# lincbrain/Fibers.jl

Measured on AMD Instinct MI355X. Metric: Mvoxels/s fit (GQI ODF + peaks, 140^3 x 270-dir); Mpoints/s streamline in extra, higher is better.
Workload: dtype f32 (operands as 2 fp16 pieces = 23 bits on MFMA, 3 piece products, f32 accumulate); 1 GPU; gqi_rec + find_peaks + qa normalisation (gqi.jl:109-201), ONE 140x140x140 x 270-frame volume (18 x b=5 + 84 dirs x {1000,2000,3000}), sphere_642, all-ones mask; voxels=2744000, voxels_per_gpu=2744000, frames=270, odf_vertices=321, parallelism=single GPU

## Files before the change

### fibers.jl_amd/csrc/odf.hip

```cpp
#include <algorithm>
#include <cmath>
#include <type_traits>
#include <utility>

#include "common.h"

namespace {

typedef float f32x16 __attribute__((ext_vector_type(16)));

constexpr int KT = 16;
constexpr int WG_VOX = 128;

#include "odf_gemm_f32.inc"
#include "odf_fused_epilogue.inc"
#include "odf_gemm3.inc"
#include "odf_mask.inc"
#include "odf_peaks.inc"
#include "odf_post.inc"

}

struct fib_odf_plan {
    int device = 0;
// ... 217 lines not shown
        for (int d = 0; d < p->maxdeg; d++) { const int32_t u = nbr32[(size_t)v * p->maxdeg + d]; if (u >= 0) mine.push_back(u); }
        for (int d = 0; d < FIB_S642_DEG; d++) if (fib_s642_nbr[v][d] < FIB_S642_NVERT) ref.push_back(fib_s642_nbr[v][d]);
        std::sort(mine.begin(), mine.end());
        if (mine != ref) p->is_s642 = false;
    }
    p->fused = p->fused_shape && p->is_s642 && p->At3f.p != nullptr;
    p->dsi2 = p->dsi2_shape && p->is_s642 && p->At3f.p != nullptr && p->At3b.p != nullptr;
    std::vector<int32_t> nbr64(nbr);
    for (auto &u : nbr64) if (u == p->rows_pad) u = p->nvert;
    if ((rc = p->nbr64.alloc(nbr64.size())) != FIB_OK) return rc;
    FIB_HIP(hipMemcpy(p->nbr64.p, nbr64.data(), nbr64.size() * sizeof(int32_t), hipMemcpyHostToDevice));
    std::vector<float> v3((size_t)p->nvert * 3, 0.0f);
    if (verts)
        for (int v = 0; v < p->nvert; v++)
            for (int c = 0; c < 3; c++) v3[3 * v + c] = verts[v + (size_t)nverts * c];
    if ((rc = p->At.alloc(At.size())) != FIB_OK) return rc;
    std::vector<uint32_t> effbits((size_t)p->Kpad / KT, 0u);
    for (int k = 0; k < K; k++) { if (frame_eff[k] != 0.0f) effbits[k / KT] |= 1u << (k % KT); else p->has_ineff = true; }
    if ((rc = p->effbits.alloc(effbits.size())) != FIB_OK) return rc;
    if ((rc = p->verts.alloc(v3.size())) != FIB_OK) return rc;
    if ((rc = p->nbr.alloc(nbr.size())) != FIB_OK) return rc;
    if ((rc = p->maxenc.alloc(4)) != FIB_OK) return rc;
    if ((rc = p->live_counts.alloc(4)) != FIB_OK) return rc;
    if ((rc = p->tickets.alloc(4)) != FIB_OK) return rc;
    FIB_HIP(hipMemset(p->tickets.p, 0, 4 * sizeof(unsigned)));
    if ((rc = p->selctr.alloc(2)) != FIB_OK) return rc;
    FIB_HIP(hipMemset(p->selctr.p, 0, 2 * sizeof(unsigned)));
    if ((rc = p->sellist.alloc(POST_SELCAP)) != FIB_OK) return rc;
    FIB_HIP(hipMemset(p->sellist.p, 0, POST_SELCAP * sizeof(unsigned long long)));
    if ((rc = p->odfmax.alloc(2)) != FIB_OK) return rc;
    FIB_HIP(hipMemcpy(p->At.p, At.data(), At.size() * sizeof(float), hipMemcpyHostToDevice));
    FIB_HIP(hipMemcpy(p->effbits.p, effbits.data(), effbits.size() * sizeof(uint32_t), hipMemcpyHostToDevice));
    FIB_HIP(hipMemcpy(p->verts.p, v3.data(), v3.size() * sizeof(float), hipMemcpyHostToDevice));
    FIB_HIP(hipMemcpy(p->nbr.p, nbr.data(), nbr.size() * sizeof(int32_t), hipMemcpyHostToDevice));
    return FIB_OK;
}

int check_plan_args(const float *bval, const float *bvec, int nvol, const float *verts, int nverts,
                    const int32_t *faces, int nfaces, fib_odf_plan **plan) {
    FIB_CHECK(plan != nullptr, FIB_ERR_INVALID, "plan output pointer is NULL");
    *plan = nullptr;
    FIB_CHECK(bval != nullptr && nvol > 0, FIB_ERR_MISSING_BVAL, "Missing b-value table from input DWI structure");
    FIB_CHECK(bvec != nullptr, FIB_ERR_MISSING_BVEC, "Missing gradient table from input DWI structure");
    FIB_CHECK(verts && faces && nverts >= 2 && nverts % 2 == 0 && nfaces > 0, FIB_ERR_INVALID, "invalid ODF tessellation");
    FIB_CHECK(nverts / 2 < 32768, FIB_ERR_UNSUPPORTED, "too many ODF vertices");
    return FIB_OK;
}

// ... 123 lines not shown

extern "C" int fib_odf_plan_matrix(const fib_odf_plan *plan, float *A, int *nrows, int *nvol, int *nvert) try {
    FIB_CHECK(plan != nullptr, FIB_ERR_INVALID, "plan is NULL");
    if (nrows) *nrows = plan->nrows;
    if (nvol) *nvol = plan->nvol;
    if (nvert) *nvert = plan->nvert;
    if (A) memcpy(A, plan->A.data(), plan->A.size() * sizeof(float));
    return FIB_OK;
} FIB_API_CATCH

namespace {

constexpr int FOLD_MB_MAX = 10;
template <int MB, int NX>
void launch_gemm(const GemmArgs &ga, unsigned grid, hipStream_t st) {
    if (ga.At3) {
        int ncu = 256, dev = 0;
        (void)hipGetDevice(&dev);
        (void)hipDeviceGetAttribute(&ncu, hipDeviceAttributeMultiprocessorCount, dev);
        GemmArgs g2 = ga;
        const int nw = 8;
        const int64_t items = fib::cdiv(ga.nvox, nw * 32) * ga.ntile_m;
        unsigned pg = (unsigned)std::min<int64_t>((int64_t)ncu * (8 / nw), items);
        pg = (pg + 7) / 8 * 8;
        auto go = [&](auto h2_) {
            constexpr bool H2 = decltype(h2_)::value;
            if (ga.fold) {
                if constexpr (MB <= FOLD_MB_MAX) hipLaunchKernelGGL((odf_gemm3_kernel<MB, NX, 8, true, false, H2>), dim3(pg), dim3(512), 0, st, g2);
                return;
            }
            if constexpr (MB == 10 && NX == 1) {
                if (ga.mean_hi) { hipLaunchKernelGGL((odf_gemm3_kernel<10, 1, 8, false, true, H2>), dim3(pg), dim3(512), 0, st, g2); return; }
            }
            hipLaunchKernelGGL((odf_gemm3_kernel<MB, NX, 8, false, false, H2>), dim3(pg), dim3(512), 0, st, g2);
        };
        if (ga.h2) go(std::true_type{}); else go(std::false_type{});
    }
    else hipLaunchKernelGGL((odf_gemm_kernel<MB, NX>), dim3(grid), dim3(256), 0, st, ga);
}

size_t peaks_smem(const fib_odf_plan *p) {
    return ((size_t)(p->rows_pad + 1) * PV + (size_t)PG * PV * PREC) * sizeof(float);
}

template <int DEG, bool EXACT>
int launch_peaks_t(const PeakArgs &pa, size_t smem, unsigned grid, hipStream_t st) {
// ... 135 lines not shown
    { const char *pi = fib::ab_env("FIBERS_PHASE_ITEM"); ga.phase_item = pi ? atoi(pi) : 2; }
    { const char *pw = fib::ab_env("FIBERS_PHASE_WG"); ga.phase_wg = pw ? atoi(pw) : 8; }
#endif
    ga.vec_ok = (nvox % 4 == 0 && ((uintptr_t)odf & 15) == 0 && (pdf == nullptr || ((uintptr_t)pdf & 15) == 0)) ? 1 : 0; ga.vidx = plan->live_vox.p; ga.nlive = plan->live_counts.p; ga.mask = mask; ga.effbits = plan->effbits.p;
    ga.out0 = pdf; ga.out1 = odf; ga.nvox = nvox;
    if (ga.At3 && plan->Gdev.p) {
        int rci = plan->inf_list.ensure((size_t)nvox);
        if (rci != FIB_OK) return rci;
        ga.fix_count = plan->live_counts.p + 2; ga.fix_list = plan->inf_list.p; ga.fix_cap = (int)std::min<int64_t>(nvox, INT32_MAX);
    }
    const bool sep = (flags & FIB_ODF_SEPARATE_PEAKS) != 0;
    const bool fuse = plan->fused && ga.At3 != nullptr && ga.vec_ok && !sep;
    {
        int rcm = plan->mean_hi.ensure((size_t)nvox + 4);
        if (rcm != FIB_OK) return rcm;
    }
    auto setup_fused = [&]() -> int {
        int rcf = plan->redo_list.ensure((size_t)nvox);
        if (rcf != FIB_OK) return rcf;
        ga.At3 = plan->At3f.p; ga.Aextra = plan->Aextraf.p;
        for (int k = 0; k < 3; k++) { ga.peak[k] = peak[k]; ga.qa[k] = qa[k]; }
        ga.verts = plan->verts.p; ga.maxenc = plan->maxenc.p; ga.mean_hi = plan->mean_hi.p;
        ga.redo_count = plan->live_counts.p + 3; ga.redo_list = plan->redo_list.p; ga.redo_cap = (int)std::min<int64_t>(nvox, INT32_MAX);
        { const char *pa = fib::ab_env("FIBERS_ODF_ANTI"); ga.anti = pa ? atoi(pa) : 3; }
        return FIB_OK;
    };
    if (fuse) { int rcf = setup_fused(); if (rcf != FIB_OK) return rcf; }
    ga.K = plan->gK; ga.Kpad = plan->Kpad; ga.M = plan->gM; ga.nrow0 = plan->gRow0; ga.ntile_m = plan->ntile_m;
    const bool fold_ok = plan->folded && ga.At3 != nullptr && plan->Kpad <= FKMAX && plan->scale_frame_raw >= 0 &&
                         (int64_t)plan->fold_span_max * nvox * 4 < (int64_t)0xE0000000ll;
    const bool fuse_fold = fold_ok && plan->MB <= FOLD_MB_MAX;
    const bool dsi2 = plan->dsi2 && fold_ok && ga.vec_ok && !sep;
    if (dsi2) {
        int rcf = setup_fused();
        if (rcf != FIB_OK) return rcf;
        ga.At3b = plan->At3b.p;
        ga.ntile_m = 2;
    }
    if (fuse_fold || dsi2) {
        ga.fold = 1;
        ga.rowA = plan->foldA.p; ga.rowB = plan->foldB.p;
    } else if (plan->folded) {
        int rcf = plan->folded_dwi.ensure((size_t)plan->gK * nvox);
        if (rcf != FIB_OK) return rcf;
        fib::ProfScope prof("dsi_fold", st);
        if (nvox % 4 == 0 && ((uintptr_t)dwi & 15) == 0 && ((uintptr_t)mask & 3) == 0)
// ... 136 lines not shown
    FIB_HIP(hipGetLastError());
    return FIB_OK;
} FIB_API_CATCH

extern "C" int fibd_qa_normalize_pair(float *const qa[3], int64_t nvox, float *odfmax_pair_dev, void *stream) try {
    FIB_CHECK(qa && qa[0] && qa[1] && qa[2] && odfmax_pair_dev && nvox > 0, FIB_ERR_INVALID, "NULL argument");
    hipLaunchKernelGGL(qa_normalize_kernel, dim3(2048), dim3(256), 0, (hipStream_t)stream, qa[0], qa[1], qa[2], nvox, odfmax_pair_dev, 0.0f, 1);
    FIB_HIP(hipGetLastError());
    return FIB_OK;
} FIB_API_CATCH

extern "C" int fibd_find_peaks(const fib_odf_plan *plan, const float *odf, int64_t nvox,
                               int32_t *isort_top, int32_t *nvalid, void *stream) try {
    FIB_CHECK(plan && odf && isort_top && nvalid && nvox > 0, FIB_ERR_INVALID, "NULL argument");
    fib::DeviceGuard guard;
    FIB_HIP(hipSetDevice(plan->device));
    return launch_peaks(plan, odf, nvox, nvox, nullptr, nullptr, isort_top, nvalid, false, (hipStream_t)stream);
} FIB_API_CATCH

#ifdef FIB_CLOCK_STAMP
extern "C" int fib_debug_clock_stamps(unsigned long long *out, int cap) try {
    FIB_CHECK(out && cap > 0 && cap <= 2048, FIB_ERR_INVALID, "invalid stamp buffer");
    FIB_HIP(hipDeviceSynchronize());
    FIB_HIP(hipMemcpyFromSymbol(out, HIP_SYMBOL(fib_clock_stamps), (size_t)cap * 4 * sizeof(unsigned long long), 0, hipMemcpyDeviceToHost));
    return FIB_OK;
} FIB_API_CATCH
extern "C" int fib_debug_phase_stamps(unsigned long long *out) try {
    FIB_CHECK(out, FIB_ERR_INVALID, "invalid stamp buffer");
    FIB_HIP(hipDeviceSynchronize());
    FIB_HIP(hipMemcpyFromSymbol(out, HIP_SYMBOL(fib_phase_stamps), sizeof(unsigned long long) * 512, 0, hipMemcpyDeviceToHost));
    return FIB_OK;
} FIB_API_CATCH

extern "C" int fib_debug_clock_clear(void) try {
    static unsigned long long zeros[2048][4];
    FIB_HIP(hipMemcpyToSymbol(HIP_SYMBOL(fib_clock_stamps), zeros, sizeof(zeros), 0, hipMemcpyHostToDevice));
    return FIB_OK;
} FIB_API_CATCH
#endif

extern "C" int fibd_find_peaks_work(const fib_odf_plan *plan, const float *odf, int64_t nvox,
                                    float *odf_peak, int32_t *isort, int32_t *nvalid, void *stream) try {
    FIB_CHECK(plan && odf && odf_peak && isort && nvalid && nvox > 0, FIB_ERR_INVALID, "NULL argument");
    FIB_CHECK(plan->nbr64.p != nullptr && plan->maxdeg > 0, FIB_ERR_INVALID, "the plan has no tessellation");
    fib::DeviceGuard guard;
    FIB_HIP(hipSetDevice(plan->device));
    const size_t smem = (size_t)plan->nvert * sizeof(unsigned long long) + (size_t)(plan->nvert + 1) * sizeof(float);
    FIB_CHECK(smem <= 64 * 1024, FIB_ERR_UNSUPPORTED, "ODF with %d vertices does not fit the peak finder's LDS", plan->nvert);
    const unsigned grid = (unsigned)std::min<int64_t>(nvox, 8192);
    hipLaunchKernelGGL(odf_peaks_work_kernel, dim3(grid), dim3(256), smem, (hipStream_t)stream, odf, nvox, nvox, plan->nvert, plan->deg_pad,
                       plan->nbr64.p, odf_peak, isort, nvalid);
    FIB_HIP(hipGetLastError());
    return FIB_OK;
} FIB_API_CATCH
```

### fibers.jl_amd/csrc/odf_fused_epilogue.inc

```

#include "sphere642_fused.inc"
#ifndef FIB_EPI_VARIANT
#define FIB_EPI_VARIANT 0
#endif
__device__ const short fib_f642_pos_vertex_dev[321] = {
#define FIB_F642_COPY(...) __VA_ARGS__
    FIB_F642_POS_LIST(FIB_F642_COPY)
};
__device__ const short fib_f642_slot_vertex_dev[2 * 161] = {
    FIB_F642_SLOT_LIST(FIB_F642_COPY)
#undef FIB_F642_COPY
};
constexpr int FQ_CAP = 10;
constexpr int FQ_LIST = FQ_CAP * 512;
constexpr int FQ_CAPB = 9;
constexpr int FQ_LISTB = FQ_CAPB * 320;
constexpr int FQ_NPOS = 320, FQ_NSLOT = 2 * 161, FQ_NV = 321;
constexpr int FQ_TABB = (2 * FQ_NPOS + FQ_NSLOT + 3 * FQ_NV) * 4 + 12;
static_assert(FQ_TABB % 16 == 0, "table block keeps the LDS carve-up 16-byte aligned");

__device__ __forceinline__ float fq_xhalf(float x, int kh) {
    const auto r = __builtin_amdgcn_permlane32_swap(__float_as_uint(x), __float_as_uint(x), false, false);
    return __uint_as_float(kh ? r[0] : r[1]);
}
__device__ __forceinline__ float fq_xhalf_max(float x) {
    const auto r = __builtin_amdgcn_permlane32_swap(__float_as_uint(x), __float_as_uint(x), false, false);
    return __builtin_fmaxf(__uint_as_float(r[0]), __uint_as_float(r[1]));
}
__device__ __forceinline__ float fq_max3(float a, float b, float c) { return __builtin_fmaxf(__builtin_fmaxf(a, b), c); }
__device__ __forceinline__ float fq_max3z(float a, float b) { return __builtin_fmaxf(__builtin_fmaxf(a, b), 0.0f); }
__device__ __forceinline__ float fq_min3(float a, float b, float c) { return __builtin_fminf(__builtin_fminf(a, b), c); }
__device__ __forceinline__ float fq_max2(float a, float b) { return __builtin_fmaxf(a, b); }

template <int NW, bool PRE = false, bool SCALE = false, bool POW2 = false, bool DRAIN = false, int TRN = 2, bool LB = false, int CAP = FQ_CAP>
__device__ __forceinline__ void gemm3_epilogue_fused(const GemmArgs &a, f32x16 (&acc)[10], float xrow, float vmax, float vnf, bool inb, bool lv,
                                                     int64_t vox, int lane, char *tr, char *lst, const uint64_t *posoff, const int *slotv, const float *vl,
                                                     unsigned &en_run, float scale = 1.0f, float xscale = 1.0f) {
    const int col = lane & 31, kh = lane >> 5;
    const float pm = fmaxf(vmax, __shfl_xor(vmax, 32));
    const float pn = vnf + __shfl_xor(vnf, 32);
    const bool nonfinite = pn != pn;
    const bool valid = lv && (pm > 0.0f || nonfinite);
    const bool refix = a.fix_list != nullptr && lv && pm == INFINITY;
    if (!PRE) xrow += __shfl_xor(xrow, 32);
    if constexpr (SCALE) {
#pragma unroll
        for (int m = 0; m < 10; m++)
#pragma unroll
            for (int r = 0; r < 16; r++) {
                if constexpr (POW2) asm("v_mul_legacy_f32 %0, %1, %2" : "=v"(acc[m][r]) : "v"(acc[m][r]), "v"(valid ? scale : 0.0f));
                else acc[m][r] = valid ? acc[m][r] * scale : 0.0f;
            }
        xrow = valid ? xrow * xscale : 0.0f;
    } else if (!__all(valid && !nonfinite)) {
#pragma unroll
        for (int m = 0; m < 10; m++)
#pragma unroll
            for (int r = 0; r < 16; r++) acc[m][r] = valid ? acc[m][r] : 0.0f;
        xrow = valid ? xrow : 0.0f;
    }
// ... 68 lines not shown
                const unsigned cw = m < 2 ? cw0 : m < 4 ? cw1 : m < 6 ? cw2 : m < 8 ? cw3 : cw4;
                unsigned byte = (cw >> (8 * (3 - (2 * (m & 1) + hb)))) & 0xffu;
#if FIB_EPI_VARIANT & 2
                {
                    const int b = 31 - __clz((int)(byte | 1u));
                    const int j = 7 - b;
                    const float x = tw[(8 * (j >> 2) + 2 * (j & 3)) * 32];
                    if (byte != 0u) { if (cnt < CAP) list_put(cnt, x, (uint32_t)(16 * m + 8 * hb + j)); cnt++; }
                    byte &= ~(1u << b);
                }
#endif
                if (__any(byte != 0u)) {
                    while (byte != 0u) {
                        const int b = 31 - __clz((int)byte);
                        byte &= ~(1u << b);
                        const int j = 7 - b;
                        const float x = tw[(8 * (j >> 2) + 2 * (j & 3)) * 32];
                        if (cnt < CAP) list_put(cnt, x, (uint32_t)(16 * m + 8 * hb + j));
                        cnt++;
                    }
                }
            }
        };
        if constexpr (DRAIN) __builtin_amdgcn_s_waitcnt(0x0F70);
        if (__all(qinb)) rows_out(std::false_type{}); else rows_out(std::true_type{});
        if (inb && kh == 0) a.out1[(int64_t)FIB_F642_POLE * a.stride + vox] = xrow;
        if (cpole) { if (cnt < CAP) list_put(cnt, xrow, 160u); cnt++; }
    }
    float vmin = INFINITY;
#if FIB_EPI_VARIANT & 1
    float vs0 = 0.0f, vs1 = 0.0f;
#pragma unroll
    for (int m = 0; m < 10; m++)
#pragma unroll
        for (int r = 0; r < 16; r += 2) {
            vmin = fq_min3(vmin, acc[m][r], acc[m][r + 1]);
            asm("v_add_f32 %0, %1, %0" : "+v"(vs0) : "v"(acc[m][r]));
            asm("v_add_f32 %0, %1, %0" : "+v"(vs1) : "v"(acc[m][r + 1]));
        }
    const float vsum = vs0 + vs1;
#else
    f32x2 vs2 = {0.0f, 0.0f};
#pragma unroll
    for (int m = 0; m < 10; m++)
#pragma unroll
        for (int r = 0; r < 16; r += 2) {
            vmin = fq_min3(vmin, acc[m][r], acc[m][r + 1]);
// ... 52 lines not shown
```

### fibers.jl_amd/csrc/odf_gemm3.inc

```

typedef __bf16 bf16x8_t __attribute__((ext_vector_type(8)));
typedef _Float16 f16x8_t __attribute__((ext_vector_type(8)));
typedef _Float16 f16x2_t __attribute__((ext_vector_type(2)));
typedef uint32_t u32x4_t __attribute__((ext_vector_type(4)));

__device__ __forceinline__ uint32_t cvt_pk_bf16(float lo, float hi) {
    uint32_t r;
    asm("v_cvt_pk_bf16_f32 %0, %1, %2" : "=v"(r) : "v"(lo), "v"(hi));
    return r;
}

constexpr int FKMAX = 512, FSMAX = FKMAX / KT;
template <int MB, int NX, int NW, bool FOLD, bool FUSE, bool H2, bool ONE = false>
constexpr int gemm3_lds_bytes() {
    constexpr bool SF = H2 && FOLD && ONE;
    return 2 * (H2 ? 2 : 3) * MB * 1024 + NW * (FUSE && !SF ? 4096 : 2048) + (NX > 0 ? (FUSE ? 2048 : 8192) : 0) +
           (FOLD ? 2 * FKMAX * 4 + 4 * FSMAX * 4 + (FUSE ? 0 : 2 * FKMAX * 4) : 0) + (FUSE ? NW * (SF ? FQ_LISTB : FQ_LIST) + FQ_TABB : 0) +
           (H2 && FUSE && !FOLD ? NW * (4096 + 512) : 0) +
           (SF ? NW * (8192 + 256) : 0);
}
template <int MB, int NX, int NW, bool FOLD = false, bool FUSE = false, bool ONE = false, bool H2 = false>
__device__ __forceinline__ void gemm3_body(const GemmArgs &a, char *lds) {
    static_assert(!FUSE || (MB == 10 && NX == 1), "the fused peak scan is generated for 10 blocks + 1 extra row");
    constexpr int NPIECE = (H2 ? 2 : 3) * MB;
    constexpr int TILEB = NPIECE * 1024;
    constexpr int NA = (NPIECE + NW - 1) / NW;
    constexpr int WGV = NW * 32;
    constexpr int NXA = NX > 0 ? NX : 1;
    constexpr int XTAB = NX > 0 ? (FUSE ? 2048 : 8192) : 0;
    constexpr int FTAB = FOLD ? 2 * FKMAX * 4 + 4 * FSMAX * 4 + (FUSE ? 0 : 2 * FKMAX * 4) : 0;
    constexpr bool SLDSF = H2 && FOLD && ONE;
    constexpr bool SLDS = (H2 && FUSE && !FOLD) || SLDSF;
    constexpr bool BOOK = SLDS && !FOLD;
    constexpr int BOOKB = BOOK ? 512 : (SLDSF ? 256 : 0);
    constexpr int BOOKV = BOOK ? 64 : 0;
    constexpr int QLIST = SLDSF ? FQ_LISTB : FQ_LIST;
    constexpr int QTAB = FUSE ? NW * QLIST + FQ_TABB : 0;
    constexpr int TRB = FUSE && !SLDSF ? 4096 : 2048;
    constexpr int SSLOT = FOLD ? 4096 : 2048;
    constexpr int NSREQ = FOLD ? 4 : 2;
    constexpr int STILE = SLDS ? NW * (2 * SSLOT + BOOKB) : 0;
    static_assert(2 * TILEB + NW * TRB + XTAB + FTAB + QTAB + STILE == gemm3_lds_bytes<MB, NX, NW, FOLD, FUSE, H2, ONE>(), "LDS carve-up");
    static_assert(gemm3_lds_bytes<MB, NX, NW, FOLD, FUSE, H2, ONE>() <= 160 * 1024, "LDS of a CU");
    uint64_t *q_posoff = reinterpret_cast<uint64_t *>(lds + 2 * TILEB + NW * TRB + XTAB + FTAB + (FUSE ? NW * QLIST : 0));
    int *q_slotv = reinterpret_cast<int *>(q_posoff + FQ_NPOS);
    float *q_vl = reinterpret_cast<float *>(q_slotv + FQ_NSLOT);
    uint32_t *f_off = reinterpret_cast<uint32_t *>(lds + 2 * TILEB + NW * TRB + XTAB);
    int32_t *f_bs = reinterpret_cast<int32_t *>(f_off + 2 * FKMAX);
    int32_t *f_row = f_bs + 4 * FSMAX;
    const int tid = threadIdx.x, lane = tid & 63;
    const int wave = __builtin_amdgcn_readfirstlane(tid >> 6);
    const int col = lane & 31, kh = lane >> 5;
    const int ntiles = a.Kpad / KT;
    const uint32_t a_off = (uint32_t)lane * 16;
    if (NX > 0) {
        float *xt = reinterpret_cast<float *>(lds + 2 * TILEB + NW * TRB);
        for (int i = tid; i < (ONE ? 1 : a.ntile_m) * NX * a.Kpad; i += NW * 64) xt[i] = a.Aextra[i];
    }
    if constexpr (FUSE) {
        for (int i = tid; i < FQ_NPOS; i += NW * 64) q_posoff[i] = (uint64_t)fib_f642_pos_vertex_dev[i] * (uint64_t)a.stride * 4u;
        for (int i = tid; i < FQ_NSLOT; i += NW * 64) q_slotv[i] = fib_f642_slot_vertex_dev[i];
        for (int i = tid; i < 3 * FQ_NV; i += NW * 64) q_vl[i] = a.verts[i];
    }
    const char *Sbase = reinterpret_cast<const char *>(a.S);
    const uint32_t row_bytes = (uint32_t)(a.stride * 4);
// ... 17 lines not shown
            f_off[side * FKMAX + J] = f >= 0 ? (uint32_t)(f - f_bs[4 * (J / KT) + 2 * side]) * row_bytes : 0xF0000000u;
            if (!FUSE) f_row[side * FKMAX + J] = f;
        }
        __syncthreads();
    }

    const int xcd = blockIdx.x & 7, wslot = blockIdx.x >> 3, nslot = gridDim.x >> 3;
    const int nlive = __builtin_amdgcn_readfirstlane(a.nlive[0]);
    const int ntile_n = (nlive + WGV - 1) / WGV;
    struct Work { int tile_m; int tile_n; bool valid; };
    auto work_at = [&](int i) {
        const int w = wslot + i * nslot;
        Work r;
        constexpr bool ONE_M = ONE || (FUSE && !FOLD);
        r.tile_m = ONE_M ? 0 : __builtin_amdgcn_readfirstlane(w % a.ntile_m);
        r.tile_n = __builtin_amdgcn_readfirstlane(ONE ? (a.one_slot + i * a.one_stride) * 8 + xcd : (ONE_M ? w : w / a.ntile_m) * 8 + xcd);
        r.valid = r.tile_n < ntile_n;
        return r;
    };
    auto vidx_at = [&](const Work &w) -> int32_t {
        const int64_t sl = (int64_t)w.tile_n * WGV + wave * 32 + col;
        return a.vidx[sl < a.nvox ? sl : a.nvox - 1];
    };
    Work cur = work_at(0);
    if (!cur.valid) return;
    int32_t vraw = vidx_at(cur);
    Work nxt = work_at(1);
    int32_t vraw_nxt = vidx_at(nxt);

    const uint32_t lds_l = (uint32_t)(uintptr_t)((const __attribute__((address_space(3))) char *)lds);
    typedef int i32x4_t __attribute__((ext_vector_type(4)));
    i32x4_t rsrcA;
    {
        const uint64_t b = reinterpret_cast<uint64_t>(a.At3);
        rsrcA[0] = (int)(uint32_t)b; rsrcA[1] = (int)(uint32_t)((b >> 32) & 0xffffu);
        rsrcA[2] = (int)((uint32_t)(ONE ? 1 : a.ntile_m) * (uint32_t)ntiles * (uint32_t)TILEB); rsrcA[3] = 0x00020000;
    }
    auto stage_A = [&](int tile_m, int t, int buf) {
        const char *g = reinterpret_cast<const char *>(a.At3) + ((size_t)tile_m * ntiles + t) * TILEB;
        char *l = lds + buf * TILEB;
#pragma unroll
        for (int i = 0; i < NA; i++) {
            int p = wave + i * NW;
            p = p < NPIECE ? p : NPIECE - 1;
            if constexpr (H2) {
                const uint32_t d = lds_l + (uint32_t)(buf * TILEB + p * 1024);
// ... 221 lines not shown
                    const int k = a.one_slot + it * a.one_stride;
                    const unsigned *flag = a.pair_flags + (blockIdx.x & 7) * 32 + k % a.dsi_na;
                    const unsigned item = (unsigned)(k / a.dsi_na) + 1u;
                    if (tid == 0) {
                        for (int spin = 0; spin < 4000; spin++) {
                            if (__hip_atomic_load(flag, __ATOMIC_RELAXED, __HIP_MEMORY_SCOPE_AGENT) >= item) break;
                            __builtin_amdgcn_s_sleep(8);
                        }
                    }
                    __syncthreads();
                }
            }
        }
        float sraw = 0.0f;
        if (a.scale_frame >= 0) sraw = *reinterpret_cast<const float *>(Sbase + (int64_t)a.scale_frame * a.stride * 4 + (uint32_t)(vox * 4));
        bool lv;
        if constexpr (BOOK) lv = inb && (book[lane] & 0xffu) != 0u;
        else lv = inb && a.mask[vox] != 0;
        bool inb_n = false; int64_t vox_n = 0; uint32_t s_off_n = 0;
        lane_state(nxt, vraw_nxt, inb_n, vox_n, s_off_n);
        if constexpr (SLDS) qoff_n = (uint32_t)__shfl((int)vox_n, 4 * (lane & 7)) * 4u;
        if constexpr (BOOK) {
            book_mask(vox_n);
            book_vidx(work_at(g / ntiles + 2));
        }
        if constexpr (SLDSF) book_vidx(work_at(g / ntiles + 2));
        for (int t = 0; t < ntiles; t++, g++) {
            const int cb = g & 1;
            const char *L = lds + cb * TILEB;
            FIB_PHASE(g / ntiles, wave, 1);
            const bool w1 = t + 1 < ntiles;
            const int tm_n = w1 ? cur.tile_m : (nxt.valid ? nxt.tile_m : cur.tile_m);
            if constexpr (SLDS) {
                if (t > 0) stage_A(tm_n, w1 ? t + 1 : 0, cb ^ 1);
                if (!(ANTI && early)) {
                    const bool in = t + 2 < ntiles;
                    split(cur.tile_m, t, g & 1, in ? t + 2 : t + 2 - ntiles, in ? qoff : qoff_n, in || nxt.valid);
                }
                FIB_PHASE(g / ntiles, wave, 2);
            } else {
            if (!(ANTI && early)) split(cur.tile_m, t);
            FIB_PHASE(g / ntiles, wave, 2);
            stage_A(tm_n, w1 ? t + 1 : 0, cb ^ 1);
            load_B(w1 ? t + 1 : 0, w1 ? s_off : s_off_n, w1 || nxt.valid);
            }
            __builtin_amdgcn_sched_barrier(0);
            FIB_PHASE(g / ntiles, wave, 3);
// ... 50 lines not shown
                        for (int x = 0; x < NXA; x++) { xfin[x] = xacc[x]; xacc[x] = 0.0f; }
                        vmax_fin = vmax; vmax = 0.0f; vnf = 0.0f;
                        kexp_fin = kexp;
                    }
                    if constexpr (SLDS) {
                        if (w1) { const bool in = t + 3 < ntiles; split(cur.tile_m, t + 1, (g + 1) & 1, in ? t + 3 : t + 3 - ntiles, in ? qoff : qoff_n, in || nxt.valid); }
                        else split(tm_n, 0, (g + 1) & 1, 2, qoff_n, nxt.valid);
                    } else {
                        split(tm_n, w1 ? t + 1 : 0);
                    }
                }
            }
            FIB_PHASE(g / ntiles, wave, 5);
            if constexpr (SLDS) { if (t > 0 || g == 0) __builtin_amdgcn_s_waitcnt(0x0F70 | NSREQ); }
            else
            __builtin_amdgcn_s_waitcnt(0x0F70);
            FIB_PHASE(g / ntiles, wave, 6);
            if constexpr (SLDS) __builtin_amdgcn_s_barrier();
            else
            __syncthreads();
            FIB_PHASE(g / ntiles, wave, 7);
        }
        if constexpr (SLDS) stage_A(nxt.valid ? nxt.tile_m : cur.tile_m, 1, (g & 1) ^ 1);
        {
            float vm = early ? vmax_fin : vmax;
            vm = max3_nan(vm, __shfl_xor(vm, 32), 0.0f);
            if (H2 && a.scale_frame < 0 && a.fix_list != nullptr && vm > 0.0f && vm < 1.17549435e-38f) vm = INFINITY;
            const float vn = vm < INFINITY ? 0.0f : __builtin_nanf("");
            const float asc = H2 ? __uint_as_float((uint32_t)(254 - (early ? kexp_fin : kexp)) << 23) * a.h2_inv_sa : 1.0f;
            if constexpr (FUSE) {
                float fscale = 1.0f;
                if (FOLD) { const float s0 = sraw < 0.0f ? 0.0f : sraw; fscale = vn != vn ? __builtin_nanf("") : 1.0f / (a.scale_coef * s0); }
                gemm3_epilogue_fused<NW, false, FOLD || H2, H2 && !FOLD, SLDS, SLDSF ? 1 : 2, SLDSF, SLDSF ? FQ_CAPB : FQ_CAP>(a, acc, early ? xfin[0] : xacc[0], vm, vn, inb, lv, vox, lane, lds + 2 * TILEB + wave * TRB,
                                                            lds + 2 * TILEB + NW * TRB + XTAB + FTAB + wave * QLIST, q_posoff, q_slotv, q_vl, en_run,
                                                            fscale * asc, fscale);
            }
            else {
                int le = lane;
                asm volatile("" : "+v"(le));
                if constexpr (SLDS) __builtin_amdgcn_s_waitcnt(0x0F70);
                if constexpr (FOLD)
                    gemm3_epilogue<MB, NX, false, 0, true, H2>(a, acc, xacc, vm, vn, inb, lv, vox, le, cur.tile_m, sraw, lds + 2 * TILEB + wave * TRB, f_row, f_row + FKMAX, asc);
                else
                    gemm3_epilogue<MB, NX, false, 0, false, H2>(a, acc, xacc, vm, vn, inb, lv, vox, le, cur.tile_m, sraw, lds + 2 * TILEB + wave * TRB, nullptr, nullptr, asc);
            }
        }
        FIB_PHASE(g / ntiles - 1, wave, 8);
        if (!nxt.valid) break;
        cur = nxt; inb = inb_n; vox = vox_n; s_off = s_off_n; qoff = qoff_n;
        nxt = work_at(g / ntiles + 1);
        if constexpr (SLDS) vraw_nxt = (int32_t)book[BOOKV + lane];
        else vraw_nxt = vidx_at(nxt);
        clear(early);
    }
    if constexpr (SLDS) __builtin_amdgcn_s_waitcnt(0x0F70);
    FIB_STAMP_END(ONE ? 8 : (FUSE ? 2 : (FOLD ? 3 : 1)), g / ntiles);
    if constexpr (FUSE) {
        for (int off = 32; off >= 1; off >>= 1) { const unsigned oth = (unsigned)__shfl_xor((int)en_run, off); en_run = oth > en_run ? oth : en_run; }
        if (lane == 0 && en_run) atomicMax(&a.maxenc[2], en_run);
    }
}

template <int MB, int NX, int NW, bool FOLD = false, bool FUSE = false, bool H2 = false>
__global__ __launch_bounds__(NW * 64, 2) void odf_gemm3_kernel(const GemmArgs a) {
    __shared__ __attribute__((aligned(16))) char lds[gemm3_lds_bytes<MB, NX, NW, FOLD, FUSE, H2>()];
    gemm3_body<MB, NX, NW, FOLD, FUSE, false, H2>(a, lds);
}

template <int MBB, bool H2>
__global__ __launch_bounds__(512, 2) void odf_dsi2_kernel(const GemmArgs a) {
    constexpr int LA_ = gemm3_lds_bytes<10, 1, 8, true, true, H2, true>(), LB_ = gemm3_lds_bytes<MBB, 0, 8, true, false, H2, true>();
    __shared__ __attribute__((aligned(16))) char lds[LA_ > LB_ ? LA_ : LB_];
    const int wslot = blockIdx.x >> 3, nslot = gridDim.x >> 3;
// ... 15 lines not shown
```

### fibers.jl_amd/csrc/odf_gemm_f32.inc

```

struct GemmArgs {
    const float *At;
    const void *At3;
    const float *S;
    const int32_t *vidx;
    const int32_t *nlive;
    const uint8_t *mask;
    const uint32_t *effbits;
    float *out0;
    float *out1;
    int64_t nvox;
    int64_t stride;
    int K, Kpad, M, nrow0, ntile_m;
    int scale_frame;
    float scale_coef;
    int has_ineff;
    const float *Aextra;
    int vec_ok;
    const int32_t *rowA, *rowB;
    int32_t *fix_count, *fix_list;
    int fix_cap;
    int fold;
    float *peak[3], *qa[3];
    const float *verts;
    unsigned *maxenc;
    float *mean_hi;
    int32_t *redo_count, *redo_list;
    int redo_cap;
    int anti;
    const void *At3b;
    int one_slot, one_stride;
    int dsi_na;
    unsigned *pair_flags;
    int pair_role;
    int h2;
    float h2_inv_sa;
    int phase_item, phase_wg;
};

#ifdef FIB_CLOCK_STAMP
__device__ unsigned long long fib_clock_stamps[2048][4];
#define FIB_STAMP_BEGIN() unsigned long long fcs_c0_, fcs_r0_; asm volatile("s_memtime %0\n\ts_memrealtime %1\n\ts_waitcnt lgkmcnt(0)" : "=s"(fcs_c0_), "=s"(fcs_r0_) :: "memory")
#define FIB_STAMP_END(kid, items)                                                                                                   \
    do {                                                                                                                            \
        unsigned long long fcs_c1_, fcs_r1_;                                                                                        \
        asm volatile("s_memtime %0\n\ts_memrealtime %1\n\ts_waitcnt lgkmcnt(0)" : "=s"(fcs_c1_), "=s"(fcs_r1_) :: "memory");          \
        if (threadIdx.x == 0 && blockIdx.x < 2048) {                                                                                \
            fib_clock_stamps[blockIdx.x][0] = fcs_c1_ - fcs_c0_; fib_clock_stamps[blockIdx.x][1] = fcs_r1_ - fcs_r0_;               \
            fib_clock_stamps[blockIdx.x][2] = (kid); fib_clock_stamps[blockIdx.x][3] = (unsigned long long)(items);                 \
        }                                                                                                                           \
    } while (0)
__device__ unsigned long long fib_phase_stamps[2][256];
#ifdef FIB_PHASE_STAMP
#define FIB_PHASE_VARS() int fps_n_ = 0
#define FIB_PHASE(item_, wave_, id_)                                                                                                \
    do {                                                                                                                            \
        if ((int)blockIdx.x == a.phase_wg && (item_) == a.phase_item && ((wave_) & 3) == 0 && fps_n_ < 256) {                                     \
            unsigned long long t_;                                                                                                  \
            asm volatile("s_memtime %0\n\ts_waitcnt lgkmcnt(0)" : "=s"(t_) :: "memory");                                          \
            if ((threadIdx.x & 63) == 0) fib_phase_stamps[(wave_) >> 2][fps_n_] = (t_ << 8) | (unsigned)(id_);                      \
            fps_n_++;                                                                                                               \
        }                                                                                                                           \
    } while (0)
#else
#define FIB_PHASE_VARS() do { } while (0)
#define FIB_PHASE(item_, wave_, id_) do { } while (0)
#endif
#else
#define FIB_STAMP_BEGIN() do { } while (0)
#define FIB_STAMP_END(kid, items) do { } while (0)
#define FIB_PHASE_VARS() do { } while (0)
#define FIB_PHASE(item_, wave_, id_) do { } while (0)
#endif

template <int MB>
__device__ __forceinline__ void interleave_ds_mfma() {
#pragma unroll
    for (int i = 0; i < MB / 2; i++) {
        __builtin_amdgcn_sched_group_barrier(0x100, 1, 0);
        __builtin_amdgcn_sched_group_barrier(0x008, 2, 0);
    }
    if (MB & 1) {
        __builtin_amdgcn_sched_group_barrier(0x100, 1, 0);
        __builtin_amdgcn_sched_group_barrier(0x008, 1, 0);
    }
}

typedef float f32x2 __attribute__((ext_vector_type(2)));

__device__ __forceinline__ float clamp_sample(float x) {
    float c;
// ... 384 lines not shown
```

### fibers.jl_amd/csrc/odf_mask.inc

```

constexpr int CB = 4096;
constexpr int CB_ITERS_MAX = 32;
__device__ __forceinline__ unsigned long long quad_expand(unsigned long long b) {
    unsigned long long q = (b | (b >> 1) | (b >> 2) | (b >> 3)) & 0x1111111111111111ull;
    return q | (q << 1) | (q << 2) | (q << 3);
}
__device__ __forceinline__ unsigned long long octet_expand(unsigned long long b) {
    return ((b & 0xffffffffull) ? 0xffffffffull : 0ull) | ((b >> 32) ? 0xffffffff00000000ull : 0ull);
}
struct ZeroArgs { float *out0, *out1, *peak[3], *qa[3]; int n0, n1; int64_t nvox, stride; };
struct CompactArgs {
    const uint8_t *mask; int64_t nvox;
    int32_t *vidx, *tiles;
    unsigned long long *state;
    unsigned *ticket;
    int32_t *totals;
    unsigned *maxenc;
    unsigned epoch;
    int nchunks, iters, zero;
    unsigned *clear; int nclear;
    unsigned long long *sub_state;
    unsigned long long *state2;
    unsigned *mode;
    int force;
// ... 86 lines not shown
            if (lane == 0 && (pv | pt)) { atomicAdd(&s_base[0], pv); atomicAdd(&s_base[1], pt); }
        }
        if (t == c.nchunks - 1 && c.state2 && c.mode) {
            int aq = 0, ao = 0;
            if (tid <= t) {
                unsigned long long g;
                for (;;) {
                    g = __hip_atomic_load((fib_gu64 *)(c.state2 + tid), __ATOMIC_RELAXED, __HIP_MEMORY_SCOPE_AGENT);
                    if ((unsigned)(g >> 36) == (c.epoch & 0xfffffffu)) break;
                    __builtin_amdgcn_s_sleep(1);
                }
                aq = (int)((g >> 18) & 0x3ffffull); ao = (int)(g & 0x3ffffull);
            }
#pragma unroll
            for (int off = 32; off >= 1; off >>= 1) { aq += __shfl_xor(aq, off); ao += __shfl_xor(ao, off); }
            if (lane == 0 && (aq | ao)) { atomicAdd(&s_altsum[0], aq); atomicAdd(&s_altsum[1], ao); }
        }
        __syncthreads();
        if (t == c.nchunks - 1 && wave == 0) {
            if (lane == 0 && c.state2 && c.mode) c.mode[(c.epoch + 1u) & 1u] = (2ll * s_altsum[1] <= 3ll * s_altsum[0]) ? 1u : 0u;
            if (lane == 0) {
                c.totals[0] = s_base[0] + s_agg[0]; c.totals[1] = s_base[1] + s_agg[1]; c.totals[2] = 0; c.totals[3] = 0;
                if (c.maxenc) { c.maxenc[0] = 0u; c.maxenc[1] = 0u; c.maxenc[2] = 0u; c.maxenc[3] = 0u; }
                c.ticket[0] = 0u; c.ticket[1] = 0u;
            }
            for (int i = lane; i < c.nclear; i += 64) c.clear[i] = 0u;
        }
        for (int it = 0; it < c.iters; it++)
#pragma unroll
            for (int i = 0; i < 4; i++) {
                const int64_t vx = base + (int64_t)it * CB + i * 1024 + tid;
                const unsigned long long b = __ballot(vx < c.nvox && c.mask[vx] != 0);
                const unsigned long long e = (oct ? octet_expand(b) : quad_expand(b)) & __ballot(vx < c.nvox);
                const int pv = s_base[0] + cv[it][i * 16 + wave], pt = s_base[1] + ct[it][i * 16 + wave];
                if ((e >> lane) & 1ull) c.vidx[pv + __popcll(e & ((1ull << lane) - 1ull))] = (int32_t)vx;
                if (lane == 0 && b) c.tiles[pt] = (int32_t)(vx >> 6);
            }
        if (!c.zero) return;
    }
    const ZeroArgs &z = c.z;
    constexpr int ZS = 8, ZR = 16;
    __shared__ int s_nd[ZS], s_known, s_tot[2];
    const int nr = z.n0 + z.n1 + 12, ngrp = (nr + ZR - 1) / ZR;
    const int64_t nsub = (c.nvox + CB - 1) / CB, nspan = (nsub + ZS - 1) / ZS;
    const int hb = (int)blockIdx.x, nh = (int)gridDim.x;
    if (tid < 2) s_tot[tid] = 0;
    __syncthreads();
// ... 207 lines not shown
```

Baseline: 1512 Mvoxels/s.

## Add dynamic work dealing via global ticket counter in fused H2 GEMM kernel

In the fused non-fold LDS-staged GEMM path, each workgroup grabs a global atomic ticket after each item and posts it to a two-slot LDS mailbox. Beyond a fixed lookahead it fetches the next tile from that ticket instead of a static stride. The ticket is read only after the epilogue's memory drain, so the atomic latency should be hidden. The aim is to balance load across workgroups with uneven per-tile cost, at the price of a global atomic per item and an extra counter reset in the mask kernel. It also adds debug stamps for entry and end times and an env knob to cap the grid size.

After: 1489 Mvoxels/s. -1.5%, worse.

```diff
diff --git a/fibers.jl_amd/csrc/odf.hip b/fibers.jl_amd/csrc/odf.hip
--- a/fibers.jl_amd/csrc/odf.hip
+++ b/fibers.jl_amd/csrc/odf.hip
@@ -263,8 +263,8 @@
     if ((rc = p->nbr.alloc(nbr.size())) != FIB_OK) return rc;
     if ((rc = p->maxenc.alloc(4)) != FIB_OK) return rc;
     if ((rc = p->live_counts.alloc(4)) != FIB_OK) return rc;
-    if ((rc = p->tickets.alloc(4)) != FIB_OK) return rc;
-    FIB_HIP(hipMemset(p->tickets.p, 0, 4 * sizeof(unsigned)));
+    if ((rc = p->tickets.alloc(8)) != FIB_OK) return rc;
+    FIB_HIP(hipMemset(p->tickets.p, 0, 8 * sizeof(unsigned)));
     if ((rc = p->selctr.alloc(2)) != FIB_OK) return rc;
     FIB_HIP(hipMemset(p->selctr.p, 0, 2 * sizeof(unsigned)));
     if ((rc = p->sellist.alloc(POST_SELCAP)) != FIB_OK) return rc;
@@ -434,6 +434,7 @@
         const int nw = 8;
         const int64_t items = fib::cdiv(ga.nvox, nw * 32) * ga.ntile_m;
         unsigned pg = (unsigned)std::min<int64_t>((int64_t)ncu * (8 / nw), items);
+        if (const char *eg = fib::ab_env("FIBERS_ODF_GRID")) { const int n = atoi(eg); if (n > 0) pg = std::min(pg, (unsigned)n); }
         pg = (pg + 7) / 8 * 8;
         auto go = [&](auto h2_) {
             constexpr bool H2 = decltype(h2_)::value;
@@ -615,6 +616,8 @@
         for (int k = 0; k < 3; k++) { ga.peak[k] = peak[k]; ga.qa[k] = qa[k]; }
         ga.verts = plan->verts.p; ga.maxenc = plan->maxenc.p; ga.mean_hi = plan->mean_hi.p;
         ga.redo_count = plan->live_counts.p + 3; ga.redo_list = plan->redo_list.p; ga.redo_cap = (int)std::min<int64_t>(nvox, INT32_MAX);
+        ga.deal = plan->tickets.p + 4;
+        { const char *pd = fib::ab_env("FIBERS_ODF_DEAL"); ga.deal_dyn = (pd && pd[0] == 's') ? 0 : 1; }
         { const char *pa = fib::ab_env("FIBERS_ODF_ANTI"); ga.anti = pa ? atoi(pa) : 3; }
         return FIB_OK;
     };
@@ -797,7 +800,16 @@
 extern "C" int fib_debug_clock_stamps(unsigned long long *out, int cap) try {
     FIB_CHECK(out && cap > 0 && cap <= 2048, FIB_ERR_INVALID, "invalid stamp buffer");
     FIB_HIP(hipDeviceSynchronize());
-    FIB_HIP(hipMemcpyFromSymbol(out, HIP_SYMBOL(fib_clock_stamps), (size_t)cap * 4 * sizeof(unsigned long long), 0, hipMemcpyDeviceToHost));
+    static unsigned long long all[2048][6];
+    FIB_HIP(hipMemcpyFromSymbol(all, HIP_SYMBOL(fib_clock_stamps), (size_t)cap * 6 * sizeof(unsigned long long), 0, hipMemcpyDeviceToHost));
+    for (int i = 0; i < cap; i++)
+        for (int j = 0; j < 4; j++) out[4 * i + j] = all[i][j];
+    return FIB_OK;
+} FIB_API_CATCH
+extern "C" int fib_debug_clock_stamps6(unsigned long long *out, int cap) try {
+    FIB_CHECK(out && cap > 0 && cap <= 2048, FIB_ERR_INVALID, "invalid stamp buffer");
+    FIB_HIP(hipDeviceSynchronize());
+    FIB_HIP(hipMemcpyFromSymbol(out, HIP_SYMBOL(fib_clock_stamps), (size_t)cap * 6 * sizeof(unsigned long long), 0, hipMemcpyDeviceToHost));
     return FIB_OK;
 } FIB_API_CATCH
 extern "C" int fib_debug_phase_stamps(unsigned long long *out) try {
@@ -808,7 +820,7 @@
 } FIB_API_CATCH
 
 extern "C" int fib_debug_clock_clear(void) try {
-    static unsigned long long zeros[2048][4];
+    static unsigned long long zeros[2048][6];
     FIB_HIP(hipMemcpyToSymbol(HIP_SYMBOL(fib_clock_stamps), zeros, sizeof(zeros), 0, hipMemcpyHostToDevice));
     return FIB_OK;
 } FIB_API_CATCH
diff --git a/fibers.jl_amd/csrc/odf_fused_epilogue.inc b/fibers.jl_amd/csrc/odf_fused_epilogue.inc
--- a/fibers.jl_amd/csrc/odf_fused_epilogue.inc
+++ b/fibers.jl_amd/csrc/odf_fused_epilogue.inc
@@ -32,10 +32,11 @@
 __device__ __forceinline__ float fq_min3(float a, float b, float c) { return __builtin_fminf(__builtin_fminf(a, b), c); }
 __device__ __forceinline__ float fq_max2(float a, float b) { return __builtin_fmaxf(a, b); }
 
-template <int NW, bool PRE = false, bool SCALE = false, bool POW2 = false, bool DRAIN = false, int TRN = 2, bool LB = false, int CAP = FQ_CAP>
+struct FqNoop { __device__ __forceinline__ void operator()() const {} };
+template <int NW, bool PRE = false, bool SCALE = false, bool POW2 = false, bool DRAIN = false, int TRN = 2, bool LB = false, int CAP = FQ_CAP, class DRAINED = FqNoop>
 __device__ __forceinline__ void gemm3_epilogue_fused(const GemmArgs &a, f32x16 (&acc)[10], float xrow, float vmax, float vnf, bool inb, bool lv,
                                                      int64_t vox, int lane, char *tr, char *lst, const uint64_t *posoff, const int *slotv, const float *vl,
-                                                     unsigned &en_run, float scale = 1.0f, float xscale = 1.0f) {
+                                                     unsigned &en_run, float scale = 1.0f, float xscale = 1.0f, DRAINED drained = DRAINED()) {
     const int col = lane & 31, kh = lane >> 5;
     const float pm = fmaxf(vmax, __shfl_xor(vmax, 32));
     const float pn = vnf + __shfl_xor(vnf, 32);
@@ -150,7 +151,7 @@
                 }
             }
         };
-        if constexpr (DRAIN) __builtin_amdgcn_s_waitcnt(0x0F70);
+        if constexpr (DRAIN) { __builtin_amdgcn_s_waitcnt(0x0F70); drained(); }
         if (__all(qinb)) rows_out(std::false_type{}); else rows_out(std::true_type{});
         if (inb && kh == 0) a.out1[(int64_t)FIB_F642_POLE * a.stride + vox] = xrow;
         if (cpole) { if (cnt < CAP) list_put(cnt, xrow, 160u); cnt++; }
diff --git a/fibers.jl_amd/csrc/odf_gemm3.inc b/fibers.jl_amd/csrc/odf_gemm3.inc
--- a/fibers.jl_amd/csrc/odf_gemm3.inc
+++ b/fibers.jl_amd/csrc/odf_gemm3.inc
@@ -16,12 +16,13 @@
     constexpr bool SF = H2 && FOLD && ONE;
     return 2 * (H2 ? 2 : 3) * MB * 1024 + NW * (FUSE && !SF ? 4096 : 2048) + (NX > 0 ? (FUSE ? 2048 : 8192) : 0) +
            (FOLD ? 2 * FKMAX * 4 + 4 * FSMAX * 4 + (FUSE ? 0 : 2 * FKMAX * 4) : 0) + (FUSE ? NW * (SF ? FQ_LISTB : FQ_LIST) + FQ_TABB : 0) +
-           (H2 && FUSE && !FOLD ? NW * (4096 + 512) : 0) +
+           (H2 && FUSE && !FOLD ? NW * (4096 + 512) + 16 : 0) +
            (SF ? NW * (8192 + 256) : 0);
 }
 template <int MB, int NX, int NW, bool FOLD = false, bool FUSE = false, bool ONE = false, bool H2 = false>
 __device__ __forceinline__ void gemm3_body(const GemmArgs &a, char *lds) {
     static_assert(!FUSE || (MB == 10 && NX == 1), "the fused peak scan is generated for 10 blocks + 1 extra row");
+    FIB_STAMP_ENTRY();
     constexpr int NPIECE = (H2 ? 2 : 3) * MB;
     constexpr int TILEB = NPIECE * 1024;
     constexpr int NA = (NPIECE + NW - 1) / NW;
@@ -40,7 +41,10 @@
     constexpr int SSLOT = FOLD ? 4096 : 2048;
     constexpr int NSREQ = FOLD ? 4 : 2;
     constexpr int STILE = SLDS ? NW * (2 * SSLOT + BOOKB) : 0;
-    static_assert(2 * TILEB + NW * TRB + XTAB + FTAB + QTAB + STILE == gemm3_lds_bytes<MB, NX, NW, FOLD, FUSE, H2, ONE>(), "LDS carve-up");
+    constexpr bool DEAL = SLDS && FUSE && !FOLD;
+    constexpr int DEAL_AHEAD = 4;
+    constexpr int MBOXB = DEAL ? 16 : 0;
+    static_assert(2 * TILEB + NW * TRB + XTAB + FTAB + QTAB + STILE + MBOXB == gemm3_lds_bytes<MB, NX, NW, FOLD, FUSE, H2, ONE>(), "LDS carve-up");
     static_assert(gemm3_lds_bytes<MB, NX, NW, FOLD, FUSE, H2, ONE>() <= 160 * 1024, "LDS of a CU");
     uint64_t *q_posoff = reinterpret_cast<uint64_t *>(lds + 2 * TILEB + NW * TRB + XTAB + FTAB + (FUSE ? NW * QLIST : 0));
     int *q_slotv = reinterpret_cast<int *>(q_posoff + FQ_NPOS);
@@ -104,6 +108,11 @@
         const int64_t sl = (int64_t)w.tile_n * WGV + wave * 32 + col;
         return a.vidx[sl < a.nvox ? sl : a.nvox - 1];
     };
+    uint32_t *mbox = reinterpret_cast<uint32_t *>(lds + 2 * TILEB + NW * TRB + XTAB + FTAB + QTAB + STILE);
+    const bool deal_dyn = DEAL && a.deal_dyn != 0;
+    const int deal_base = DEAL_AHEAD * (int)gridDim.x;
+    uint32_t ticket = 0u;
+    Work ahead{};
     Work cur = work_at(0);
     if (!cur.valid) return;
     int32_t vraw = vidx_at(cur);
@@ -371,7 +380,16 @@
         if constexpr (SLDS) qoff_n = (uint32_t)__shfl((int)vox_n, 4 * (lane & 7)) * 4u;
         if constexpr (BOOK) {
             book_mask(vox_n);
-            book_vidx(work_at(g / ntiles + 2));
+            if constexpr (DEAL) {
+                const int it = g / ntiles;
+                ahead = work_at(it + 2);
+                if (deal_dyn && it + 2 >= DEAL_AHEAD) {
+                    ahead.tile_n = __builtin_amdgcn_readfirstlane((int)mbox[it & 1]);
+                    ahead.valid = ahead.tile_n < ntile_n;
+                }
+                book_vidx(ahead);
+            }
+            else book_vidx(work_at(g / ntiles + 2));
         }
         if constexpr (SLDSF) book_vidx(work_at(g / ntiles + 2));
         for (int t = 0; t < ntiles; t++, g++) {
@@ -468,6 +486,17 @@
             FIB_PHASE(g / ntiles, wave, 7);
         }
         if constexpr (SLDS) stage_A(nxt.valid ? nxt.tile_m : cur.tile_m, 1, (g & 1) ^ 1);
+        if constexpr (DEAL) {
+            if (wave == 0 && lane == 0) asm volatile("global_atomic_add %0, %1, %2, off sc0" : "=v"(ticket) : "v"(a.deal), "v"(1u) : "memory");
+        }
+        auto deal_put = [&]() {
+            if constexpr (DEAL) {
+                if (wave == 0 && lane == 0) {
+                    asm volatile("; ticket landed" : "+v"(ticket) :: "memory");
+                    mbox[(g / ntiles - 1) & 1] = ticket + (uint32_t)deal_base;
+                }
+            }
+        };
         {
             float vm = early ? vmax_fin : vmax;
             vm = max3_nan(vm, __shfl_xor(vm, 32), 0.0f);
@@ -479,7 +508,7 @@
                 if (FOLD) { const float s0 = sraw < 0.0f ? 0.0f : sraw; fscale = vn != vn ? __builtin_nanf("") : 1.0f / (a.scale_coef * s0); }
                 gemm3_epilogue_fused<NW, false, FOLD || H2, H2 && !FOLD, SLDS, SLDSF ? 1 : 2, SLDSF, SLDSF ? FQ_CAPB : FQ_CAP>(a, acc, early ? xfin[0] : xacc[0], vm, vn, inb, lv, vox, lane, lds + 2 * TILEB + wave * TRB,
                                                             lds + 2 * TILEB + NW * TRB + XTAB + FTAB + wave * QLIST, q_posoff, q_slotv, q_vl, en_run,
-                                                            fscale * asc, fscale);
+                                                            fscale * asc, fscale, deal_put);
             }
             else {
                 int le = lane;
@@ -494,7 +523,8 @@
         FIB_PHASE(g / ntiles - 1, wave, 8);
         if (!nxt.valid) break;
         cur = nxt; inb = inb_n; vox = vox_n; s_off = s_off_n; qoff = qoff_n;
-        nxt = work_at(g / ntiles + 1);
+        if constexpr (DEAL) nxt = ahead;
+        else nxt = work_at(g / ntiles + 1);
         if constexpr (SLDS) vraw_nxt = (int32_t)book[BOOKV + lane];
         else vraw_nxt = vidx_at(nxt);
         clear(early);
diff --git a/fibers.jl_amd/csrc/odf_gemm_f32.inc b/fibers.jl_amd/csrc/odf_gemm_f32.inc
--- a/fibers.jl_amd/csrc/odf_gemm_f32.inc
+++ b/fibers.jl_amd/csrc/odf_gemm_f32.inc
@@ -35,11 +35,14 @@
     int pair_role;
     int h2;
     float h2_inv_sa;
+    unsigned *deal;
+    int deal_dyn;
     int phase_item, phase_wg;
 };
 
 #ifdef FIB_CLOCK_STAMP
-__device__ unsigned long long fib_clock_stamps[2048][4];
+__device__ unsigned long long fib_clock_stamps[2048][6];
+#define FIB_STAMP_ENTRY() unsigned long long fcs_e_; asm volatile("s_memrealtime %0\n\ts_waitcnt lgkmcnt(0)" : "=s"(fcs_e_) :: "memory")
 #define FIB_STAMP_BEGIN() unsigned long long fcs_c0_, fcs_r0_; asm volatile("s_memtime %0\n\ts_memrealtime %1\n\ts_waitcnt lgkmcnt(0)" : "=s"(fcs_c0_), "=s"(fcs_r0_) :: "memory")
 #define FIB_STAMP_END(kid, items)                                                                                                   \
     do {                                                                                                                            \
@@ -48,6 +51,7 @@
         if (threadIdx.x == 0 && blockIdx.x < 2048) {                                                                                \
             fib_clock_stamps[blockIdx.x][0] = fcs_c1_ - fcs_c0_; fib_clock_stamps[blockIdx.x][1] = fcs_r1_ - fcs_r0_;               \
             fib_clock_stamps[blockIdx.x][2] = (kid); fib_clock_stamps[blockIdx.x][3] = (unsigned long long)(items);                 \
+            fib_clock_stamps[blockIdx.x][4] = fcs_e_; fib_clock_stamps[blockIdx.x][5] = fcs_r1_;                                     \
         }                                                                                                                           \
     } while (0)
 __device__ unsigned long long fib_phase_stamps[2][256];
@@ -67,6 +71,7 @@
 #define FIB_PHASE(item_, wave_, id_) do { } while (0)
 #endif
 #else
+#define FIB_STAMP_ENTRY() do { } while (0)
 #define FIB_STAMP_BEGIN() do { } while (0)
 #define FIB_STAMP_END(kid, items) do { } while (0)
 #define FIB_PHASE_VARS() do { } while (0)
diff --git a/fibers.jl_amd/csrc/odf_mask.inc b/fibers.jl_amd/csrc/odf_mask.inc
--- a/fibers.jl_amd/csrc/odf_mask.inc
+++ b/fibers.jl_amd/csrc/odf_mask.inc
@@ -132,7 +132,7 @@
             if (lane == 0) {
                 c.totals[0] = s_base[0] + s_agg[0]; c.totals[1] = s_base[1] + s_agg[1]; c.totals[2] = 0; c.totals[3] = 0;
                 if (c.maxenc) { c.maxenc[0] = 0u; c.maxenc[1] = 0u; c.maxenc[2] = 0u; c.maxenc[3] = 0u; }
-                c.ticket[0] = 0u; c.ticket[1] = 0u;
+                c.ticket[0] = 0u; c.ticket[1] = 0u; c.ticket[4] = 0u;
             }
             for (int i = lane; i < c.nclear; i += 64) c.clear[i] = 0u;
         }
```
